# AlerianEmperor/CaitlynRenderer

Measured on AMD Instinct MI355X. Metric: Mray/s (primary+1 bounce) at 1920x1080, higher is better.
Workload: dtype f32

## Files before the change

### caitlynrenderer_amd/csrc/crt_device.cpp

```cpp
#include <hip/hip_runtime.h>
#include <dlfcn.h>

#include <algorithm>
#include <atomic>
#include <chrono>
#include <cmath>
#include <cstdio>
#include <cstdlib>
#include <cstring>
#include <memory>
#include <mutex>
#include <thread>
#include <new>
#include <string>
#include <vector>

#include "../../include/crt.h"
#include "crt_error.hpp"
#include "device_build.hpp"
#include "host/cwbvh.hpp"
#include "host/flatnode_link.hpp"
#include "host/refit_core.hpp"
#include "instances.hpp"
#include "instances_bind.hpp"
// ... 426 lines not shown
}

static int init_scene_common(crt_scene* s, const crt_scene_desc* d) {
    if (hipGetDevice(&s->device) != hipSuccess) return (fail(CRT_ERR_HIP, "hipGetDevice failed"));
    hipDeviceProp_t prop;
    if (hipGetDeviceProperties(&prop, s->device) == hipSuccess) s->n_cu = prop.multiProcessorCount;
    if (const char* e = std::getenv("CRT_TIMING")) s->timing = (uint32_t)std::max(0, std::atoi(e));
    if (hipStreamCreateWithFlags(&s->stream, hipStreamNonBlocking) != hipSuccess) return (fail(CRT_ERR_HIP, "hipStreamCreate failed"));
    s->width = d->width; s->height = d->height; s->max_depth = d->max_depth; s->n_lights = (uint32_t)d->n_lights;
    s->n_vertices = d->n_vertices; s->n_normals = d->n_normals; s->n_slots = d->n_triangles;
    if (d->n_vertices) {
        for (int k = 0; k < 3; ++k) s->bounds_lo[k] = s->bounds_hi[k] = d->vertices[k];
        for (size_t i = 1; i < d->n_vertices; ++i)
            for (int k = 0; k < 3; ++k) {
                s->bounds_lo[k] = std::min(s->bounds_lo[k], d->vertices[3 * i + k]);
                s->bounds_hi[k] = std::max(s->bounds_hi[k], d->vertices[3 * i + k]);
            }
    }
    for (size_t m = 0; m < d->n_materials; ++m)
        s->special_materials = s->special_materials || d->materials[m].albedo[3] == 1.0f || d->materials[m].albedo[3] == 17.0f;
    return CRT_OK;
}

static void note_buf(crt_scene* s, const void* member, size_t bytes) {
    s->scene_bufs.emplace_back((size_t)(reinterpret_cast<const char*>(member) - reinterpret_cast<const char*>(s)), bytes);
}

template <typename T>
static int pad_rows(crt_scene* s, T** buf, uint32_t rows_in, uint32_t rows_out, size_t n_items) {
    if (rows_in == rows_out || !*buf) return CRT_OK;
    T* padded = nullptr;
    int rc = dev_alloc(&padded, n_items * rows_out);
    if (rc) return rc;
    crt::launch_restride(*buf, rows_in, padded, rows_out, n_items, s->stream);
    if (hipStreamSynchronize(s->stream) != hipSuccess || hipGetLastError() != hipSuccess) { (void)hipFree(padded); return fail(CRT_ERR_HIP, "crt_scene_create: re-striding failed"); }
    (void)hipFree(*buf);
    *buf = padded;
    return CRT_OK;
}

static int ensure_planes(crt_scene* s) {
    if (s->d_planes || !s->d_nodes || !s->info.n_nodes8) return CRT_OK;
    int rc;
    if (s->primary && s->shares_scene) {
        crt_scene* const p = s->primary;
        if ((rc = ensure_planes(p))) return rc;
// ... 311 lines not shown
    } else if (!nodes8) {
        if (!conv.convert(d->bvh, d->n_bvh, d->n_triangles, d->tri_orig_ids))
            return fail(CRT_ERR_INVALID, "crt_scene_create: BVH2 -> CWBVH failed: " + conv.error);
        nodes8 = conv.nodes.data(); n_nodes8 = conv.nodes.size();
        tri_slots = conv.tri_slots.data(); n_tris8 = conv.tri_slots.size();
    } else if (!tri_slots) {
        return fail(CRT_ERR_INVALID, "crt_scene_create: bvh8 given without bvh8_tri_slots");
    }
    {
        std::string why = crt::validate_cwbvh(nodes8, n_nodes8, n_tris8, CRT_STACK_ENTRIES, &depth8);
        if (!why.empty()) return fail(why.find("deeper") != std::string::npos ? CRT_ERR_LIMIT : CRT_ERR_INVALID,
                                      "crt_scene_create: CWBVH rejected: " + why);
        for (size_t i = 0; i < n_tris8; ++i)
            if (tri_slots[i] < 0 || (size_t)tri_slots[i] >= d->n_triangles)
                return fail(CRT_ERR_INVALID, "crt_scene_create: bvh8_tri_slots entry out of range");
    }

    if (n_nodes8 * (uint64_t)(CRT_NODE_ROWS * 16) >= (1ull << 32) || n_tris8 * (uint64_t)(CRT_TRI_ROWS * 16) >= (1ull << 32))
        return fail(CRT_ERR_LIMIT, "crt_scene_create: CWBVH node or triangle-record array of 4 GiB or more (53 M nodes / 89 M records)");
    std::unique_ptr<crt_scene> owner(new (std::nothrow) crt_scene);
    crt_scene* s = owner.get();
    if (!s) return fail(CRT_ERR_NOMEM, "crt_scene_create: out of memory");
    auto bail = [&](int code) { return code; };
    if ((rc = init_scene_common(s, d))) return bail(rc);
    s->stack_entries = std::min<uint32_t>(CRT_STACK_ENTRIES, std::max<uint32_t>(2, depth8 - 1u));
    s->info.n_nodes8 = n_nodes8; s->info.n_tris8 = n_tris8; s->info.n_bvh2_nodes = d->n_bvh; s->info.max_depth8 = depth8;

    std::vector<float4> recs(3 * n_tris8);
    for (size_t i = 0; i < n_tris8; ++i) {
        const int32_t slot = tri_slots[i];
        const crt_triangle& t = d->triangles[slot];
        const float* v0 = d->vertices + 3 * (size_t)t.v[0];
        const float* v1 = d->vertices + 3 * (size_t)t.v[1];
        const float* v2 = d->vertices + 3 * (size_t)t.v[2];
        const int32_t id = d->tri_orig_ids ? d->tri_orig_ids[slot] : slot;
        float4 a, b, c;
        a.x = v0[0]; a.y = v0[1]; a.z = v0[2]; std::memcpy(&a.w, &id, 4);
        b.x = v1[0] - v0[0]; b.y = v1[1] - v0[1]; b.z = v1[2] - v0[2]; std::memcpy(&b.w, &slot, 4);
        c.x = v2[0] - v0[0]; c.y = v2[1] - v0[1]; c.z = v2[2] - v0[2]; std::memcpy(&c.w, &t.v[3], 4);
        recs[3 * i] = a; recs[3 * i + 1] = b; recs[3 * i + 2] = c;
    }

#define UP(dst, src, count, T)                                                                             \
    do {                                                                                                   \
        if ((rc = dev_alloc(&(dst), (count)))) return bail(rc);                                            \
        if ((count) && hipMemcpy((dst), (src), (count) * sizeof(T), hipMemcpyHostToDevice) != hipSuccess)  \
            return bail(fail(CRT_ERR_HIP, "hipMemcpy H2D failed"));                                        \
// ... 60 lines not shown
    note_buf(s, &s->d_normals, d->n_normals * 3 * sizeof(float));
    note_buf(s, &s->d_materials, d->n_materials * sizeof(crt_material));
    note_buf(s, &s->d_lights, d->n_lights * sizeof(crt_light));
    if (have_tex) {
        note_buf(s, &s->d_texcoords, d->n_texcoords * sizeof(float2));
        note_buf(s, &s->d_textures, (size_t)d->tex_width * d->tex_height * d->n_textures * 3 * sizeof(float));
    }
    if (d->bvh) {
        note_buf(s, &s->d_bvh2, d->n_bvh * sizeof(crt_flatnode));
        note_buf(s, &s->d_tris2, d->n_triangles * 3 * sizeof(float4));
    }
    if ((rc = finish_scene_setup(s))) return bail(rc);
    *out = owner.release();
    return CRT_OK;
}

static int scene_create_device_built(const crt_scene_desc* d, crt_scene** out) {
    const auto t_begin = std::chrono::steady_clock::now();
    if (2ull * d->n_triangles >= crt::kMaxLinkBits) return fail(CRT_ERR_LIMIT, "crt_scene_create: more than 2^29 triangles");
    const bool have_tex = d->albedo_textures && d->n_textures > 0;
    std::unique_ptr<crt_scene> owner(new (std::nothrow) crt_scene);
    crt_scene* s = owner.get();
    if (!s) return fail(CRT_ERR_NOMEM, "crt_scene_create: out of memory");
    int rc = init_scene_common(s, d);
    if (rc) return rc;
    const uint32_t n = (uint32_t)d->n_triangles, n2 = 2u * n - 1u;
    hipStream_t st = s->stream;

    crt::DeviceArena arena;
    auto P = crt::DeviceArena::padded;
    const uint32_t gpu_build_flags = (d->build_flags & CRT_BUILD_SAH) ? (CRT_GPU_BUILD_SAH | (d->build_flags & 0xff00u))
                                     : (d->build_flags & CRT_BUILD_PLOC) ? (CRT_GPU_BUILD_PLOC | (d->build_flags & 0xff00u)) : 0u;
    const size_t tmp_bytes = std::max(crt::lbvh_tmp_bytes(n, gpu_build_flags), crt::cwbvh_tmp_bytes(n2, n));
    hipError_t he = arena.reserve(P((size_t)n * sizeof(crt_triangle)) + P(4) + P((size_t)n * 4) + P((size_t)n * 4) + tmp_bytes);
    if (he != hipSuccess) return fail(CRT_ERR_NOMEM, std::string("crt_scene_create: hipMalloc: ") + hipGetErrorString(he));
    crt_triangle* d_in = arena.take<crt_triangle>(n);
    uint32_t* d_flag = arena.take<uint32_t>(1);
    uint32_t* d_tri_order = arena.take<uint32_t>(n);
    int32_t* d_tri_slots = arena.take<int32_t>(n);
    const size_t persistent_mark = arena.used;

#define UPA(dst, src, count, T)                                                                                      \
    do {                                                                                                             \
        if ((rc = dev_alloc(&(dst), (count)))) return rc;                                                            \
        if ((count) && hipMemcpyAsync((dst), (src), (count) * sizeof(T), hipMemcpyHostToDevice, st) != hipSuccess)   \
            return fail(CRT_ERR_HIP, "hipMemcpy H2D failed");                                                        \
    } while (0)
// ... 1550 lines not shown
```

### caitlynrenderer_amd/csrc/rt_kernels.hip

```cpp
#include <hip/hip_runtime.h>
#include <hip/hip_ext.h>
#include <stdint.h>

#include <type_traits>
#include <stdlib.h>

#include <algorithm>

#include "rt_kernels.hpp"
#include "rt_math.hpp"
#include "host/flatnode_link.hpp"
#include "rt_traverse.hpp"

namespace crt {

#define CRT_INF 1e9f
#define CRT_EPS 1e-4f
#define CRT_PI 3.1415926f
#define CRT_PI2 6.2831853f


#ifdef CRT_ISA_MARKS
#define CRT_MARK(name) asm volatile("; CRT_MARK " name)
#else
#define CRT_MARK(name) ((void)0)
#endif

__device__ __forceinline__ void count_wave_step(uint32_t& c) {
    const unsigned long long m = __ballot(true);
    if ((int)(threadIdx.x & 63u) == __builtin_ctzll(m)) ++c;
}

__device__ unsigned long long* g_step_hist = nullptr;
__device__ uint32_t g_step_hist_mode = 0u;
__device__ __forceinline__ void hist_node_step(bool any, uint32_t nidx = 0u, uint32_t oct = 0u) {
    unsigned long long* const h = g_step_hist;
    if (h == nullptr) return;
    const unsigned long long m = __ballot(true);
    uint32_t n = (uint32_t)__builtin_popcountll(m);
    if (g_step_hist_mode) {
        const uint32_t key = (nidx << 3) | (oct & 7u);
        unsigned long long left = m;
        n = 0u;
        while (left) {
            const uint32_t k0 = (uint32_t)__shfl((int)key, __builtin_ctzll(left));
            left &= ~__ballot(key == k0);
            ++n;
        }
// ... 849 lines not shown
        const uint32_t v = static_chunk<true>(wid, nullptr, a.n, it);
        if (v == CRT_NO_WORK) break;
        const uint32_t i = dense_item(v, wave, lane);
        if (i >= a.n) continue;
        const float4 r0 = a.rays[2 * (size_t)i], r1 = a.rays[2 * (size_t)i + 1];
        HitState best;
        uint32_t nn = 0, nt = 0;
        const bool hit = traverse_bvh2<ANY, STATS>(a.nodes, a.tris, V3(r0.x, r0.y, r0.z), V3(r1.x, r1.y, r1.z), r0.w, a.tie, stk,
                                                   (int)a.stack_entries, a.overflow, best, nn, nt);
        float4 h;
        h.x = ANY ? 0.f : (hit ? best.t : 0.f);
        h.y = ANY ? 0.f : best.u;
        h.z = ANY ? 0.f : best.v;
        h.w = __int_as_float(ANY ? (hit ? 0 : -1) : best.id);
        a.hits[i] = h;
        if (STATS) a.stats[i] = ((nt > 65535u ? 65535u : nt) << 16) | (nn > 65535u ? 65535u : nn);
    }
}


__device__ __forceinline__ uint32_t wave_append(bool want, uint32_t* counter) {
    const unsigned long long m = __ballot(want);
    if (m == 0ull) return 0u;
    const uint32_t lane = threadIdx.x & 63u;
    const int leader = __builtin_ctzll(m);
    uint32_t base = 0;
    if ((int)lane == leader) base = atomicAdd(counter, (uint32_t)__builtin_popcountll(m));
    base = __shfl(base, leader);
    return base + (uint32_t)__builtin_popcountll(m & ((1ull << lane) - 1ull));
}

#include "rt_sort.hpp"

__device__ __forceinline__ uint32_t here(uint32_t uniform) { asm volatile("" : "+s"(uniform)); return uniform; }

__device__ __forceinline__ bool pixel_of(const FrameArgs& f, uint32_t i, uint32_t& px, uint32_t& py) {
    uint32_t t, bx, by;
    const uint32_t k = i & 63u;
    if (f.tile_log2) {
        const uint32_t s2 = 2u * f.tile_log2, sb = f.tile_log2 - 3u;
        t = i >> s2;
        const uint32_t blk = (i & ((1u << s2) - 1u)) >> 6;
        bx = blk & ((1u << sb) - 1u); by = blk >> sb;
    } else {
        const uint32_t tile_px = here(f.tile * f.tile);
        t = i / tile_px;
        const uint32_t blk = (i - t * tile_px) >> 6, blocks_per_row = here(f.tile >> 3);
        by = blk / blocks_per_row; bx = blk - by * blocks_per_row;
    }
    const uint2 txy = f.tile_xy[t];
    px = txy.x * f.tile + bx * 8u + (k & 7u);
    py = txy.y * f.tile + by * 8u + (k >> 3);
    return px < f.width && py < f.height;
}

__device__ __forceinline__ int wrap_i(int i, int n) { const int m = i % n; return m < 0 ? m + n : m; }
__device__ __forceinline__ vec3 sample_albedo(const SegmentArgs& a, float u, float v, int layer) {
    const int W = a.tex_width, H = a.tex_height;
    layer = layer < 0 ? 0 : layer > a.n_textures - 1 ? a.n_textures - 1 : layer;
    const float* img = a.textures + (size_t)layer * (size_t)W * (size_t)H * 3;
    const float x = u * (float)W - 0.5f, y = v * (float)H - 0.5f;
    float x0 = __builtin_floorf(x), y0 = __builtin_floorf(y);
    float fx = x - x0, fy = y - y0;
    if (!(__builtin_fabsf(x0) < 1e9f)) { x0 = 0.f; fx = 0.f; }
    if (!(__builtin_fabsf(y0) < 1e9f)) { y0 = 0.f; fy = 0.f; }
    const int i0 = wrap_i((int)x0, W), i1 = wrap_i((int)x0 + 1, W);
    const int j0 = wrap_i((int)y0, H), j1 = wrap_i((int)y0 + 1, H);
// ... 130 lines not shown
    b.ovf_base = k->bins_out.ovf_base; b.per_lane = k->bins_out.per_lane;
    for (int i = 0; i < 3; ++i) { b.origin[i] = k->bins_out.origin[i]; b.scale[i] = k->bins_out.scale[i]; }
    return b;
}
__device__ __forceinline__ KArgs kernarg_here() {
    KArgs p = (KArgs)__builtin_amdgcn_kernarg_segment_ptr();
    asm volatile("" : "+s"(p));
    return p;
}

#ifndef CRT_SEG_OCC
#define CRT_SEG_OCC 6
#endif
#ifndef CRT_SEG_OCC_DEFERRED
#define CRT_SEG_OCC_DEFERRED 8
#endif
#ifndef CRT_SEG_OCC_FIRST
#define CRT_SEG_OCC_FIRST 6
#endif
#ifndef CRT_SEG_OCC_BATCH
#define CRT_SEG_OCC_BATCH 5
#endif

template <bool FIRST, bool STATS, bool TEX, bool PRETRACED, bool INPLACE, bool BVH2 = false, bool MAT = false, bool BATCH = false, bool WIDE = false, bool ONE = false,
          bool INST = false>
__global__ void __launch_bounds__(CRT_TRACE_BLOCK, ((WIDE || ONE) ? CRT_SEG_OCC_FIRST : (BATCH || STATS) ? CRT_SEG_OCC_BATCH : (!FIRST && !INPLACE && !PRETRACED) ? CRT_SEG_OCC_DEFERRED : CRT_SEG_OCC)) k_segment(std::conditional_t<INST, InstSegmentArgs, SegmentArgs> a) {
    extern __shared__ uint2 s_lds[];
    constexpr bool UNI_K = FIRST;
    const bool wave_samples = BATCH && !WIDE && !ONE && a.wave_samples == 1u;
    const bool lane_samples = BATCH && (ONE || a.wave_samples == 2u);
    const WaveId wid = wave_id(wave_samples, lane_samples);
    const uint32_t lane = wid.lane, wave = wid.wave;
    const uint32_t wave_stride = (a.stack_entries + CRT_HIT_SLOTS) * 64u;
    uint2* stk = s_lds + (size_t)wid.lds_wave * wave_stride + lane;
    int* stk2 = reinterpret_cast<int*>(s_lds) + (size_t)wid.lds_wave * a.stack_entries2 * 64u + lane;
    const float4* const recs = BVH2 ? a.tris2 : a.tris;
    const FrameArgs& f = a.f;
    uint32_t nn = 0, nt = 0, nn_any = 0, nt_any = 0;
    uint32_t wn = 0, wt = 0, wn_any = 0, wt_any = 0;
    uint32_t n_hits = 0;
    uint32_t nu = 0, nu_any = 0;
    if (FIRST && a.zero_counts && blockIdx.x == 0)
        for (uint32_t i = threadIdx.x; i < a.n_zero; i += blockDim.x) a.zero_counts[i] = 0u;
    CRT_CHUNK_LOOP(it) {
        uint32_t v;
        if (!FIRST && a.bin_start) {
            const uint32_t n_chunks = queue_chunks(a.count_in[0]), per_group = (n_chunks + 7u) >> 3;
            const uint32_t grp = wid.vblock & 7u, c = (wid.vblock >> 3) + it * (wid.vgrid >> 3);
            v = (c < per_group && grp * per_group + c < n_chunks) ? (grp << 28) | (grp * per_group + c) : CRT_NO_WORK;
        } else {
            v = static_chunk<FIRST>(wid, a.count_in, f.n_local_pixels, it);
        }
        if (v == CRT_NO_WORK) break;
        const uint32_t g = v >> 28;
        uint32_t* const count_shadow = a.count_shadow + g * CRT_COUNTER_STRIDE;
        uint32_t* const count_next = a.count_next + g * CRT_COUNTER_STRIDE;
        float4* const shadow_q = a.shadow + 2 * (size_t)g * a.sub_capacity;
        float4* const next_q = a.rays_next + 2 * (size_t)g * a.sub_capacity;
        uint32_t e, n;
        uint32_t cost_tile = 0;
        bool cost_valid = false;
        uint32_t cost_t0 = 0;
        if (FIRST) {
            e = dense_item(v, wave, lane);
            if (lane_samples) {
                const uint32_t j = lane & 15u, q = wid.quadrant;
                e = dense_item(v, wave, 0u) + (((q >> 1) * 4u + (j >> 2)) * 8u + (q & 1u) * 4u + (j & 3u));
            }
            n = f.n_local_pixels;
            if (f.tile_order && e < n) {
                const uint32_t tile_px = f.tile * f.tile;
                const uint32_t slot = f.tile_log2 ? e >> (2u * f.tile_log2) : e / here(tile_px);
                cost_tile = f.tile_order[slot];
                e = cost_tile * tile_px + (e - slot * tile_px);
            }
            if (a.tile_cost) cost_t0 = __builtin_amdgcn_readfirstlane((uint32_t)__builtin_readcyclecounter());
            cost_tile = __builtin_amdgcn_readlane(cost_tile, 0);
            cost_valid = __builtin_amdgcn_readlane((uint32_t)(e < n), 0) != 0u;
        } else {
            e = ((v & 0x0fffffffu) * 4u + wave) * 64u + lane;
            n = a.bin_start ? a.count_in[0] : a.count_in[g * CRT_COUNTER_STRIDE];
        }
        const uint32_t ws_waves = blockDim.x >> 6;
        const uint32_t n_smp = (ONE || !BATCH) ? 1u : (wave_samples ? (a.n_samples + ws_waves - 1u) / ws_waves : lane_samples ? a.n_samples >> 2 : a.n_samples);
        const uint32_t e_of_chunk = e;
        for (uint32_t smp_it = 0; smp_it < n_smp; ++smp_it) {
        if (BATCH) { e = e_of_chunk; asm volatile("" : "+v"(e)); }
        const uint32_t smp = wave_samples ? smp_it * ws_waves + wid.lds_wave : lane_samples ? smp_it * 4u + (lane >> 4) : smp_it;
        float rv = BATCH ? a.rv_s[smp & 7u] : f.rv;
        if (lane_samples) {
            rv = a.rv_s[0];
            for (uint32_t k = 1; k < 8u; ++k) rv = smp == k ? a.rv_s[k] : rv;
        }
        bool active = e < n && (!wave_samples || smp < a.n_samples);
        uint32_t pix = 0;
        vec3 o = V3(0.f, 0.f, 0.f), d = V3(0.f, 0.f, 1.f);
        vec3 L = V3(0.f, 0.f, 0.f), T = V3(1.f, 1.f, 1.f);
        float prev_pdf = 1.0f, sx = 0.f, sy = 0.f;
        bool is_specular = true, true_area = false;
        uint32_t slot_mask = 0u;
        if (FIRST) {
            uint32_t px = 0, py = 0;
            pix = BATCH ? smp * f.n_local_pixels + e : e;
            active = active && pixel_of(f, e, px, py);
            sx = (float)px + 0.5f; sy = (float)py + 0.5f;
            const float W = (float)here(f.width), H = (float)here(f.height);
            float jx = 0.f, jy = 0.f;
            if (f.jitter) {
                const float r1 = 2.0f * shader_rand(sx, sy, rv);
                const float r2 = 2.0f * shader_rand(sx, sy, rv);
                jx = r1 < 1.0f ? sqrt_ieee(r1) - 1.0f : 1.0f - sqrt_ieee(2.0f - r1);
                jy = r2 < 1.0f ? sqrt_ieee(r2) - 1.0f : 1.0f - sqrt_ieee(2.0f - r2);
                jx = __fdiv_rn(jx, W * 0.5f);
                jy = __fdiv_rn(jy, H * 0.5f);
            }
            const float tx = __fdiv_rn((float)px + 0.5f, W), ty = __fdiv_rn((float)py + 0.5f, H);
            float dx = (2.0f * tx - 1.0f) + jx;
            float dy = (2.0f * ty - 1.0f) + jy;
            dx = dx * f.aspect_tan;
            dy = dy * f.tan_fov;
            const vec3 right = V3(f.cam_right[0], f.cam_right[1], f.cam_right[2]);
            const vec3 up = V3(f.cam_up[0], f.cam_up[1], f.cam_up[2]);
            const vec3 fwd = V3(f.cam_forward[0], f.cam_forward[1], f.cam_forward[2]);
            d = normalize((right * dx + up * dy) + fwd);
            o = V3(f.cam_pos[0], f.cam_pos[1], f.cam_pos[2]);
        } else if (active) {
            const float4* rq;
            if (a.bin_start) {
                CRT_MARK("loop_begin bins");
                rq = a.rays_in + 2 * (size_t)binned_entry(a.bin_start, a.bin_off_in, a.ovf_base_in, e);
                CRT_MARK("loop_end");
            } else {
                rq = a.rays_in + 2 * ((size_t)g * a.sub_capacity + e);
            }
            const float4 r0 = rq[0], r1 = rq[1];
            o = V3(r0.x, r0.y, r0.z); d = V3(r1.x, r1.y, r1.z);
            pix = __float_as_uint(r1.w);
        }

        HitState hit;
        hit.tri = -1;
        if (PRETRACED) {
            if (active) {
                const float4 h = a.hits_in[(size_t)g * a.sub_capacity + e];
                hit.t = h.x; hit.u = h.y; hit.v = h.z; hit.tri = __float_as_int(h.w);
            }
        } else if (BVH2) {
            if (active) traverse_bvh2<false, STATS>(a.nodes2, a.tris2, o, d, CRT_INF, a.tie, stk2, (int)a.stack_entries2, a.overflow, hit, nn, nt);
// ... 13 lines not shown
                for (uint32_t k = 1; k < 8u; ++k) rv = smp_of == k ? ka->rv_s[k] : rv;
            }
            const float4 Tp = ka->pb.T[pix];
            const float2 sd = ka->pb.seed[pix];
            if (INPLACE) { const float4 Lp = ka->pb.L[pix]; L = V3(Lp.x, Lp.y, Lp.z); prev_pdf = Lp.w; }
            else prev_pdf = ka->pb.L[pix].w;
            T = V3(Tp.x, Tp.y, Tp.z);
            is_specular = (__float_as_uint(Tp.w) & 1u) != 0u;
            true_area = (__float_as_uint(Tp.w) & 2u) != 0u;
            slot_mask = __float_as_uint(Tp.w) & 0xffffff00u;
            sx = sd.x; sy = sd.y;
        }
        auto contribute = [&](vec3 c) {
            if (INPLACE) L = L + c;
            else { ka->contrib[pix] = make_float4(c.x, c.y, c.z, 1.0f); slot_mask |= ka->slot_bit; }
        };
        bool emit_shadow = false, emit_next = false, finished = active, pending = false;
        float pend_pdf = 0.f;
        float4 sh0 = make_float4(0, 0, 0, 0), sh1 = sh0, sh2 = sh0, nx0 = sh0, nx1 = sh0;
        if (active && hit.tri >= 0) {
            CRT_MARK("shade_begin");
            if (STATS) ++n_hits;
            const float t = hit.t, bu = hit.u, bv = hit.v;
            const size_t rec_rows = BVH2 ? 3u : (size_t)CRT_TRI_ROWS;
            int slot, mtl;
            uint32_t inst_word = 0u, inst_id = 0u, normal0 = 0u, texcoord0 = 0u;
            if constexpr (INST) {
                inst_id = (uint32_t)a.hit_inst[(size_t)g * ka->sub_capacity + e];
                const uint2 iw = a.inst_mesh[inst_id];
                inst_word = iw.x;
                const uint4 mb = a.mesh_base[inst_word & 0x7fffffffu];
                slot = (int)mb.x + hit.tri;
                mtl = ka->triangles[3 * (size_t)slot].w + (int)iw.y;
                normal0 = mb.y; texcoord0 = mb.z;
            } else {
                const float4 tb = recs[rec_rows * (size_t)hit.tri + 1], tc = recs[rec_rows * (size_t)hit.tri + 2];
                slot = __float_as_int(tb.w); mtl = __float_as_int(tc.w);
            }
            int4 vn = ka->triangles[3 * (size_t)slot + 1];
            if constexpr (INST) { if (vn.w != 0) { vn.x += (int)normal0; vn.y += (int)normal0; vn.z += (int)normal0; } }
            vec3 n;
            if (vn.w == 0) n = V3((float)vn.x, (float)vn.y, (float)vn.z);
            else {
                const float* N = ka->normals;
                const vec3 na = V3(N[3 * (size_t)vn.x], N[3 * (size_t)vn.x + 1], N[3 * (size_t)vn.x + 2]);
                const vec3 nb = V3(N[3 * (size_t)vn.y], N[3 * (size_t)vn.y + 1], N[3 * (size_t)vn.y + 2]);
                const vec3 nc = V3(N[3 * (size_t)vn.z], N[3 * (size_t)vn.z + 1], N[3 * (size_t)vn.z + 2]);
                const float w = 1.0f - bu - bv;
                n = (na * w + nb * bu) + nc * bv;
            }
            if constexpr (INST) {
                if ((inst_word & 0x80000000u) == 0u) {
                    const float* W = a.inst_w2o + 12 * (size_t)inst_id;
                    vec3 m = V3((W[0] * n.x + W[4] * n.y) + W[8] * n.z, (W[1] * n.x + W[5] * n.y) + W[9] * n.z, (W[2] * n.x + W[6] * n.y) + W[10] * n.z);
                    const float ln = sqrt_ieee((n.x * n.x + n.y * n.y) + n.z * n.z), lm = sqrt_ieee((m.x * m.x + m.y * m.y) + m.z * m.z);
                    if (lm != 0.0f && __builtin_isfinite(lm)) m = m * __fdiv_rn(ln, lm);
                    n = m;
                }
            }
            const float4 m_albedo = ka->materials[4 * (size_t)mtl], m_emission = ka->materials[4 * (size_t)mtl + 1],
                         m_specular = ka->materials[4 * (size_t)mtl + 2];
            const float cos_incident = dot(d, n);
            const vec3 original_n = n;
            if (cos_incident > 0) n = -n;
            if (m_emission.w != -1.0f) {
                const vec3 em = V3(m_emission.x, m_emission.y, m_emission.z);
                if (is_specular) contribute(T * em);
                else {
                    vec3 ld = d * t;
                    const float len = length(ld);
                    ld = normalize(ld);
                    const float cos_light = -1.0f * dot(ld, n);
                    const float len2 = len * len;
                    const int li = (int)m_emission.w;
                    const float* ap = ka->lights + 18 * (size_t)li + 15;
                    float pdf_light = __fdiv_rn(len2, ap[0] * cos_light) * ap[1];
                    if (MAT && true_area) pdf_light = 2.0f * pdf_light;
                    const float tt = prev_pdf * prev_pdf;
                    const float w = __fdiv_rn(tt, pdf_light * pdf_light + tt);
                    contribute((T * em) * w);
                }
            } else {
                const vec3 hit_point = (o + d * t) + n * 0.0002f;
                vec3 albedo = V3(m_albedo.x, m_albedo.y, m_albedo.z);
                if (TEX) {
                    const float tex = ka->materials[4 * (size_t)mtl + 3].x;
                    if (tex != -1.0f && ka->textures != nullptr) {
                        int4 vt = ka->triangles[3 * (size_t)slot + 2];
                        if constexpr (INST) { vt.x += (int)texcoord0; vt.y += (int)texcoord0; vt.z += (int)texcoord0; }
                        const float2 ta = ka->texcoords[vt.x], tb2 = ka->texcoords[vt.y], tc2 = ka->texcoords[vt.z];
                        const float w = 1.0f - bu - bv;
                        const float tu = (ta.x * w + tb2.x * bu) + tc2.x * bv;
                        const float tv = (ta.y * w + tb2.y * bu) + tc2.y * bv;
                        const vec3 c = sample_albedo(a, tu, tv, (int)tex);
                        albedo = V3((float)pow((double)c.x, (double)2.2f), (float)pow((double)c.y, (double)2.2f),
                                    (float)pow((double)c.z, (double)2.2f));
                    }
                }
                const float mtype = m_albedo.w;
                if (MAT && mtype == CRT_MIRROR_TYPE) {
                    const vec3 ns = normalize(n);
                    const float dn = dot(d, ns);
                    T = T * albedo;
                    if (!ka->last_segment) {
                        const vec3 rdir = d - ns * (2.0f * dn);
                        if (INPLACE || FIRST) ka->pb.L[pix] = make_float4(L.x, L.y, L.z, prev_pdf);
                        ka->pb.T[pix] = make_float4(T.x, T.y, T.z, __uint_as_float(1u | slot_mask));
                        ka->pb.seed[pix] = make_float2(sx, sy);
                        emit_next = true;
                        finished = false;
                        nx0 = make_float4(hit_point.x, hit_point.y, hit_point.z, CRT_INF);
                        nx1 = make_float4(rdir.x, rdir.y, rdir.z, __uint_as_float(pix));
                    }
                } else {
                    const bool disney = MAT && mtype == CRT_DISNEY_TYPE;
                    vec3 ns = n;
                    const vec3 wo = -d;
                    Disney dm;
                    if (disney) { ns = normalize(n); dm = disney_params(albedo, m_specular.x, m_specular.y); }
                    if (m_specular.w == 0.0f) {
                        if (ka->n_lights <= 0) {
                            shader_rand(sx, sy, rv); shader_rand(sx, sy, rv); shader_rand(sx, sy, rv);
                        } else {
                            int li = (int)(shader_rand(sx, sy, rv) * (float)(int)here((uint32_t)ka->n_lights));
                            if (li > ka->n_lights - 1) li = ka->n_lights - 1;
                            const float* Lt = ka->lights + 18 * (size_t)li;
                            const float sq = sqrt_ieee(shader_rand(sx, sy, rv));
                            const float b0 = 1.0f - sq;
                            const float b1 = shader_rand(sx, sy, rv) * sq;
                            const vec3 lp = (V3(Lt[0], Lt[1], Lt[2]) + V3(Lt[3], Lt[4], Lt[5]) * b0) + V3(Lt[6], Lt[7], Lt[8]) * b1;
                            vec3 ldir = lp - hit_point;
                            const float len = length(ldir);
                            const float ilen = rcp_ieee(len);
                            ldir = ldir * ilen;
                            const float cos_mtl = dot(ldir, original_n);
                            const float cos_light = dot(ldir, V3(Lt[9], Lt[10], Lt[11]));
                            bool lit = cos_mtl > 0.0f && cos_light < 0.0f;
                            if (disney) lit = lit && dot(ns, ldir) > 0.0f;
                            if (lit) {
                                const vec3 le = V3(Lt[12], Lt[13], Lt[14]);
                                float pdf_light = __fdiv_rn(len * len, Lt[15] * -cos_light) * Lt[16];
                                vec3 c;
                                if (disney) {
                                    pdf_light = 2.0f * pdf_light;
                                    vec3 fr; float pdf_b;
                                    disney_eval(dm, ns, wo, ldir, fr, pdf_b);
                                    const float tt = pdf_light * pdf_light;
                                    const float w = __fdiv_rn(tt, pdf_b * pdf_b + tt);
                                    c = ((T * le) * fr) * (dot(ns, ldir) * w);
                                } else {
                                    const float bsdf_pdf = __fdiv_rn(dot(ldir, n) * 1.0f, CRT_PI);
                                    const float tt = pdf_light * pdf_light;
                                    const float w = __fdiv_rn(tt, bsdf_pdf * bsdf_pdf + tt);
                                    c = ((T * le) * albedo) * w;
                                }
                                c = V3(__fdiv_rn(c.x, pdf_light), __fdiv_rn(c.y, pdf_light), __fdiv_rn(c.z, pdf_light));
                                if (INPLACE) {
                                    const unsigned long long m = __ballot(true);
                                    if ((int)lane == __builtin_ctzll(m)) atomicAdd(count_shadow, (uint32_t)__builtin_popcountll(m));
                                    pending = true;
                                    sh2 = make_float4(c.x, c.y, c.z, 0.f);
                                } else {
                                    emit_shadow = true;
                                    contribute(c);
                                }
                                sh0 = make_float4(hit_point.x, hit_point.y, hit_point.z, len - CRT_EPS);
                                sh1 = make_float4(ldir.x, ldir.y, ldir.z, __uint_as_float(INPLACE ? pix : ka->slot_first + pix));
                            }
                        }
                    }
                    if (!ka->last_segment) {
                        vec3 sdir;
                        float bsdf_pdf;
                        bool go_on = true;
                        if (disney) {
                            const float u0 = shader_rand(sx, sy, rv);
                            const float u1 = shader_rand(sx, sy, rv);
                            const float u2 = shader_rand(sx, sy, rv);
                            sdir = disney_sample(dm, ns, wo, u0, u1, u2);
                            vec3 fr;
                            disney_eval(dm, ns, wo, sdir, fr, bsdf_pdf);
                            go_on = bsdf_pdf > 0.0f;
                            if (go_on) T = T * (fr * __fdiv_rn(dot(ns, sdir), bsdf_pdf));
                        } else {
                            vec3 ou, ov;
                            onb(n, ou, ov);
                            const float u1 = shader_rand(sx, sy, rv);
                            const float u2 = shader_rand(sx, sy, rv);
                            const float r = sqrt_ieee(u1);
                            const float phi = CRT_PI2 * u2;
                            const vec3 dl = V3(r * pinned_cos(phi), r * pinned_sin(phi), sqrt_ieee(1.0f - u1));
                            sdir = (ou * dl.x + ov * dl.y) + n * dl.z;
                            bsdf_pdf = __fdiv_rn(dot(sdir, n) * 1.0f, CRT_PI);
                            T = T * albedo;
                        }
                        if (go_on) {
                            if (INPLACE && pending) pend_pdf = bsdf_pdf;
                            else if (INPLACE || FIRST) ka->pb.L[pix] = make_float4(L.x, L.y, L.z, bsdf_pdf);
                            else reinterpret_cast<float*>(ka->pb.L + pix)[3] = bsdf_pdf;
                            ka->pb.T[pix] = make_float4(T.x, T.y, T.z, __uint_as_float((disney ? 2u : 0u) | slot_mask));
                            ka->pb.seed[pix] = make_float2(sx, sy);
                            emit_next = true;
                            finished = false;
                            nx0 = make_float4(hit_point.x, hit_point.y, hit_point.z, CRT_INF);
                            nx1 = make_float4(sdir.x, sdir.y, sdir.z, __uint_as_float(pix));
                        }
                    }
                }
            }
        }
        if (ka->bins_out.count) {
            const RayBins bins_out = load_bins(ka);
            CRT_MARK("loop_begin bins");
            uint32_t* const tab = wave_stride * 8u >= 3072u ? reinterpret_cast<uint32_t*>(s_lds + (size_t)wid.lds_wave * wave_stride) : nullptr;
            const uint32_t ni = bin_append(bins_out, emit_next, ray_bin_key(bins_out, nx0, nx1), tab);
            if (emit_next) { ka->rays_next[2 * (size_t)ni] = nx0; ka->rays_next[2 * (size_t)ni + 1] = nx1; }
            CRT_MARK("loop_end");
        } else {
            const uint32_t ni = wave_append(emit_next, count_next);
            if (emit_next) { next_q[2 * (size_t)ni] = nx0; next_q[2 * (size_t)ni + 1] = nx1; }
        }
        if (INPLACE) {
            const bool lanes_walks = !BVH2 && (ONE || (a.lanes_log2 != 0u && a.tri_min != 0u));
            if (FIRST && lanes_walks) {
                const bool occluded = traverse_any_then_groups<STATS, UNI_K>(a.nodes, a.tris, stk - lane, (int)a.stack_entries, a.overflow, pending, V3(sh0.x, sh0.y, sh0.z),
                                                                      V3(sh1.x, sh1.y, sh1.z), sh0.w, a.tri_min, a.lanes_log2, nn_any, nt_any, wn_any, wt_any, &nu_any, a.planes);
                if (pending && !occluded) L = L + V3(sh2.x, sh2.y, sh2.z);
            } else if (lanes_walks) {
                HitState shh;
                walk_batch<true, STATS, false, UNI_K>(a.nodes, a.tris, stk - lane, (int)a.stack_entries, a.overflow, pending, V3(sh0.x, sh0.y, sh0.z), V3(sh1.x, sh1.y, sh1.z),
                                               sh0.w, a.tri_min, a.lanes_log2, shh, nn_any, nt_any, wn_any, wt_any, V3(0.f, 0.f, 0.f), &nu_any, a.planes);
                if (pending && shh.tri < 0) L = L + V3(sh2.x, sh2.y, sh2.z);
            } else if (pending) {
                HitState sh;
                const vec3 so = V3(sh0.x, sh0.y, sh0.z), sd = V3(sh1.x, sh1.y, sh1.z);
                const bool occluded = BVH2
                    ? traverse_bvh2<true, STATS>(a.nodes2, a.tris2, so, sd, sh0.w, a.tie, stk2, (int)a.stack_entries2, a.overflow, sh, nn_any, nt_any)
                    : traverse<true, STATS, UNI_K>(a.nodes, a.tris, so, sd, sh0.w, stk, (int)a.stack_entries, a.overflow, sh, nn_any, nt_any, wn_any, wt_any, &nu_any);
                if (!occluded) L = L + V3(sh2.x, sh2.y, sh2.z);
            }
            if (pending && emit_next) a.pb.L[pix] = make_float4(L.x, L.y, L.z, pend_pdf);
            pending = false;
        } else {
// ... 379 lines not shown
```

### caitlynrenderer_amd/csrc/rt_math.hpp

```cpp
#pragma once
#include <hip/hip_runtime.h>
#include <stdint.h>

namespace crt {

struct vec3 { float x, y, z; };

__device__ __forceinline__ vec3 V3(float x, float y, float z) { return vec3{x, y, z}; }
__device__ __forceinline__ vec3 operator+(vec3 a, vec3 b) { return {a.x + b.x, a.y + b.y, a.z + b.z}; }
__device__ __forceinline__ vec3 operator-(vec3 a, vec3 b) { return {a.x - b.x, a.y - b.y, a.z - b.z}; }
__device__ __forceinline__ vec3 operator*(vec3 a, vec3 b) { return {a.x * b.x, a.y * b.y, a.z * b.z}; }
__device__ __forceinline__ vec3 operator*(vec3 a, float s) { return {a.x * s, a.y * s, a.z * s}; }
__device__ __forceinline__ vec3 operator-(vec3 a) { return {-a.x, -a.y, -a.z}; }
__device__ __forceinline__ float dot(vec3 a, vec3 b) { return (a.x * b.x + a.y * b.y) + a.z * b.z; }
__device__ __forceinline__ vec3 cross(vec3 a, vec3 b) {
    return {a.y * b.z - a.z * b.y, a.z * b.x - a.x * b.z, a.x * b.y - a.y * b.x};
}
#if defined(__gfx950__)
#define CRT_FAST_RCP 1
#else
#define CRT_FAST_RCP 0
#endif
__device__ __forceinline__ float sqrt_ieee(float x) {
#if CRT_FAST_RCP
// ... 44 lines not shown
    p = fma_add_const(p, z, -1.0 / 1307674368000.0);
    p = fma_add_const(p, z, 1.0 / 6227020800.0);
    p = fma_add_const(p, z, -1.0 / 39916800.0);
    p = fma_add_const(p, z, 1.0 / 362880.0);
    p = fma_add_const(p, z, -1.0 / 5040.0);
    p = fma_add_const(p, z, 1.0 / 120.0);
    p = fma_add_const(p, z, -1.0 / 6.0);
    return __builtin_fma(r * z, p, r);
}
__device__ __forceinline__ double cos_poly(double r) {
    double z = r * r;
    double p = z * (1.0 / 1124000727777607680000.0) + (-1.0 / 2432902008176640000.0);
    p = fma_add_const(p, z, 1.0 / 6402373705728000.0);
    p = fma_add_const(p, z, -1.0 / 20922789888000.0);
    p = fma_add_const(p, z, 1.0 / 87178291200.0);
    p = fma_add_const(p, z, -1.0 / 479001600.0);
    p = fma_add_const(p, z, 1.0 / 3628800.0);
    p = fma_add_const(p, z, -1.0 / 40320.0);
    p = fma_add_const(p, z, 1.0 / 720.0);
    p = fma_add_const(p, z, -1.0 / 24.0);
    p = fma_add_const(p, z, 0.5);
    return __builtin_fma(-z, p, 1.0);
}
__device__ __forceinline__ float pinned_sin(float xf) {
    double x = (double)xf;
    if (!(__builtin_fabs(x) < 1e9)) return 0.0f;
    double k, r = reduce_pi(x, k);
    double s = sin_poly(r);
    if (((long long)k) & 1) s = -s;
    return (float)s;
}
__device__ __forceinline__ float pinned_cos(float xf) {
    double x = (double)xf;
    if (!(__builtin_fabs(x) < 1e9)) return 1.0f;
    double k, r = reduce_pi(x, k);
    double c = cos_poly(r);
    if (((long long)k) & 1) c = -c;
    return (float)c;
}

__device__ __forceinline__ float shader_rand(float& sx, float& sy, float rv) {
    sx -= rv;
    sy -= rv;
    float d = sx * 12.9898f + sy * 78.233f;
    float v = pinned_sin(d) * 43758.5453f;
    return v - __builtin_floorf(v);
}

}
```

### caitlynrenderer_amd/csrc/rt_traverse.hpp

```cpp
#pragma once
#include <hip/hip_runtime.h>
#include <stdint.h>

#include "rt_kernels.hpp"
#include "rt_math.hpp"

namespace crt {

__device__ __forceinline__ uint32_t sign_extend_s8x4(uint32_t x) { return ((x >> 7) & 0x01010101u) * 0xffu; }


__device__ __forceinline__ float ubyte_f(uint32_t x, int j) { return (float)((x >> (8 * j)) & 0xffu); }

__device__ __forceinline__ uint32_t node8_intersect(const uint4 n0, const uint4 n1, const uint4 n2, const uint4 n3,
                                                    const uint4 n4, vec3 o, vec3 inv, bool negx, bool negy, bool negz,
                                                    uint32_t oct4, float max_t, uint32_t keep = 0xffu) {
    const vec3 p = V3(__uint_as_float(n0.x), __uint_as_float(n0.y), __uint_as_float(n0.z));
    const uint32_t e_imask = n0.w;
    const vec3 adj_inv = V3(__uint_as_float((e_imask & 0xffu) << 23) * inv.x,
                            __uint_as_float(((e_imask >> 8) & 0xffu) << 23) * inv.y,
                            __uint_as_float(((e_imask >> 16) & 0xffu) << 23) * inv.z);
    const vec3 adj_o = (p - o) * inv;
    uint32_t hit_mask = 0;
#pragma unroll
// ... 39 lines not shown
    const vec3 v0 = V3(a.x, a.y, a.z), e1 = V3(b.x, b.y, b.z), e2 = V3(c.x, c.y, c.z);
    const vec3 pv = cross(d, e2);
    const vec3 tv = o - v0;
    const vec3 qv = cross(tv, e1);
    float uu = dot(tv, pv);
    float vv = dot(d, qv);
    float tt = dot(e2, qv);
    const float inv_det = rcp_ieee(dot(e1, pv));
    uu = uu * inv_det;
    vv = vv * inv_det;
    tt = tt * inv_det;
    const float w = 1.0f - uu - vv;
    u = uu; v = vv; t = tt;
    return (uu >= 0.0f) & (vv >= 0.0f) & (tt >= 0.0f) & (w >= 0.0f);
}

__device__ __forceinline__ const uint4* node_rows(const uint4* nodes, uint32_t idx) {
    return reinterpret_cast<const uint4*>(reinterpret_cast<const char*>(nodes) + (size_t)(idx * (uint32_t)(CRT_NODE_ROWS * 16)));
}
__device__ __forceinline__ const float4* tri_rows(const float4* tris, uint32_t idx) {
    return reinterpret_cast<const float4*>(reinterpret_cast<const char*>(tris) + (size_t)(idx * (uint32_t)(CRT_TRI_ROWS * 16)));
}

#define CRT_COUNTER_STRIDE 32u


#ifdef CRT_EXPERIMENTS
#define CRT_CHUNK_LOOP(it) for (uint32_t it = 0;; ++it)
#else
#define CRT_CHUNK_LOOP(it) for (uint32_t it = 0; it < 1u; ++it)
#endif
#define CRT_NO_WORK 0xffffffffu

__device__ __forceinline__ uint32_t dense_chunks_of_group(uint32_t n_items, uint32_t g) {
    const uint32_t n_units = (((n_items + 63u) >> 6) + 63u) >> 6;
    return n_units > g ? ((n_units - g + 7u) >> 3) * 16u : 0u;
}
__device__ __forceinline__ uint32_t queue_chunks(uint32_t n) { return (((n + 63u) >> 6) + 3u) >> 2; }

struct WaveId { uint32_t lane, wave, lds_wave, vblock, vgrid, quadrant, sub; };
__device__ __forceinline__ WaveId wave_id(bool one_batch_per_workgroup = false, bool four_per_batch = false, uint32_t sub_log2 = 0u) {
    WaveId w;
    w.lane = threadIdx.x & 63u;
    w.lds_wave = threadIdx.x >> 6;
    w.sub = 0u;
    if (four_per_batch) {
// ... 52 lines not shown
```

Measured before the change: 17230.

## Tighten shading address math, skip append on last segment, add ISA marks

```diff
diff --git a/caitlynrenderer_amd/csrc/crt_device.cpp b/caitlynrenderer_amd/csrc/crt_device.cpp
--- a/caitlynrenderer_amd/csrc/crt_device.cpp
+++ b/caitlynrenderer_amd/csrc/crt_device.cpp
@@ -472,6 +472,14 @@
     return CRT_OK;
 }
 
+static int shading_arrays_addressable(const crt_scene_desc* d) {
+    const uint64_t limit = 1ull << 32;
+    if ((uint64_t)d->n_triangles * sizeof(crt_triangle) >= limit || (uint64_t)d->n_triangles * (CRT_TRI_ROWS * 16) >= limit ||
+        (uint64_t)d->n_normals * 12u >= limit || (uint64_t)d->n_materials * sizeof(crt_material) >= limit || (uint64_t)d->n_lights * sizeof(crt_light) >= limit)
+        return fail(CRT_ERR_LIMIT, "crt_scene_create: triangle, normal, material or light array of 4 GiB or more (89 M triangles, 357 M normals, 67 M materials, 59 M lights)");
+    return CRT_OK;
+}
+
 static void note_buf(crt_scene* s, const void* member, size_t bytes) {
     s->scene_bufs.emplace_back((size_t)(reinterpret_cast<const char*>(member) - reinterpret_cast<const char*>(s)), bytes);
 }
@@ -829,7 +837,7 @@
     crt_scene* s = owner.get();
     if (!s) return fail(CRT_ERR_NOMEM, "crt_scene_create: out of memory");
     auto bail = [&](int code) { return code; };
-    if ((rc = init_scene_common(s, d))) return bail(rc);
+    if ((rc = shading_arrays_addressable(d)) || (rc = init_scene_common(s, d))) return bail(rc);
     s->stack_entries = std::min<uint32_t>(CRT_STACK_ENTRIES, std::max<uint32_t>(2, depth8 - 1u));
     s->info.n_nodes8 = n_nodes8; s->info.n_tris8 = n_tris8; s->info.n_bvh2_nodes = d->n_bvh; s->info.max_depth8 = depth8;
 
@@ -936,7 +944,8 @@
     std::unique_ptr<crt_scene> owner(new (std::nothrow) crt_scene);
     crt_scene* s = owner.get();
     if (!s) return fail(CRT_ERR_NOMEM, "crt_scene_create: out of memory");
-    int rc = init_scene_common(s, d);
+    int rc = shading_arrays_addressable(d);
+    if (!rc) rc = init_scene_common(s, d);
     if (rc) return rc;
     const uint32_t n = (uint32_t)d->n_triangles, n2 = 2u * n - 1u;
     hipStream_t st = s->stream;
diff --git a/caitlynrenderer_amd/csrc/rt_kernels.hip b/caitlynrenderer_amd/csrc/rt_kernels.hip
--- a/caitlynrenderer_amd/csrc/rt_kernels.hip
+++ b/caitlynrenderer_amd/csrc/rt_kernels.hip
@@ -22,8 +22,12 @@
 
 #ifdef CRT_ISA_MARKS
 #define CRT_MARK(name) asm volatile("; CRT_MARK " name)
+#define CRT_MARK_PIN(name, x) asm volatile("; CRT_MARK " name : "+v"(x))
+#define CRT_MARK_EXPR(name, x) ({ asm volatile("; CRT_MARK " name); (x); })
 #else
 #define CRT_MARK(name) ((void)0)
+#define CRT_MARK_PIN(name, x) ((void)0)
+#define CRT_MARK_EXPR(name, x) (x)
 #endif
 
 __device__ __forceinline__ void count_wave_step(uint32_t& c) {
@@ -919,12 +923,15 @@
 __device__ __forceinline__ uint32_t wave_append(bool want, uint32_t* counter) {
     const unsigned long long m = __ballot(want);
     if (m == 0ull) return 0u;
+    CRT_MARK("cold_begin queue_append");
     const uint32_t lane = threadIdx.x & 63u;
     const int leader = __builtin_ctzll(m);
     uint32_t base = 0;
     if ((int)lane == leader) base = atomicAdd(counter, (uint32_t)__builtin_popcountll(m));
     base = __shfl(base, leader);
-    return base + (uint32_t)__builtin_popcountll(m & ((1ull << lane) - 1ull));
+    const uint32_t at = base + (uint32_t)__builtin_popcountll(m & ((1ull << lane) - 1ull));
+    CRT_MARK("cold_end");
+    return at;
 }
 
 #include "rt_sort.hpp"
@@ -940,6 +947,7 @@
         const uint32_t blk = (i & ((1u << s2) - 1u)) >> 6;
         bx = blk & ((1u << sb) - 1u); by = blk >> sb;
     } else {
+        CRT_MARK("cold npot_tiles");
         const uint32_t tile_px = here(f.tile * f.tile);
         t = i / tile_px;
         const uint32_t blk = (i - t * tile_px) >> 6, blocks_per_row = here(f.tile >> 3);
@@ -1116,6 +1124,13 @@
 #define CRT_SEG_OCC_BATCH 5
 #endif
 
+__device__ __forceinline__ float shell_rand(float& sx, float& sy, float rv) {
+    CRT_MARK_PIN("rng_begin", sx);
+    float r = shader_rand(sx, sy, rv);
+    CRT_MARK_PIN("rng_end", r);
+    return r;
+}
+
 template <bool FIRST, bool STATS, bool TEX, bool PRETRACED, bool INPLACE, bool BVH2 = false, bool MAT = false, bool BATCH = false, bool WIDE = false, bool ONE = false,
           bool INST = false>
 __global__ void __launch_bounds__(CRT_TRACE_BLOCK, ((WIDE || ONE) ? CRT_SEG_OCC_FIRST : (BATCH || STATS) ? CRT_SEG_OCC_BATCH : (!FIRST && !INPLACE && !PRETRACED) ? CRT_SEG_OCC_DEFERRED : CRT_SEG_OCC)) k_segment(std::conditional_t<INST, InstSegmentArgs, SegmentArgs> a) {
@@ -1134,8 +1149,11 @@
     uint32_t wn = 0, wt = 0, wn_any = 0, wt_any = 0;
     uint32_t n_hits = 0;
     uint32_t nu = 0, nu_any = 0;
-    if (FIRST && a.zero_counts && blockIdx.x == 0)
+    if (FIRST && a.zero_counts && blockIdx.x == 0) {
+        CRT_MARK("cold_begin zero_counts");
         for (uint32_t i = threadIdx.x; i < a.n_zero; i += blockDim.x) a.zero_counts[i] = 0u;
+        CRT_MARK("cold_end");
+    }
     CRT_CHUNK_LOOP(it) {
         uint32_t v;
         if (!FIRST && a.bin_start) {
@@ -1164,7 +1182,7 @@
             n = f.n_local_pixels;
             if (f.tile_order && e < n) {
                 const uint32_t tile_px = f.tile * f.tile;
-                const uint32_t slot = f.tile_log2 ? e >> (2u * f.tile_log2) : e / here(tile_px);
+                const uint32_t slot = f.tile_log2 ? e >> (2u * f.tile_log2) : CRT_MARK_EXPR("cold npot_tiles", e / here(tile_px));
                 cost_tile = f.tile_order[slot];
                 e = cost_tile * tile_px + (e - slot * tile_px);
             }
@@ -1182,7 +1200,10 @@
         if (BATCH) { e = e_of_chunk; asm volatile("" : "+v"(e)); }
         const uint32_t smp = wave_samples ? smp_it * ws_waves + wid.lds_wave : lane_samples ? smp_it * 4u + (lane >> 4) : smp_it;
         float rv = BATCH ? a.rv_s[smp & 7u] : f.rv;
-        if (lane_samples) {
+        if (ONE) {
+            const float rv_lo = (lane & 16u) ? a.rv_s[1] : a.rv_s[0], rv_hi = (lane & 16u) ? a.rv_s[3] : a.rv_s[2];
+            rv = (lane & 32u) ? rv_hi : rv_lo;
+        } else if (lane_samples) {
             rv = a.rv_s[0];
             for (uint32_t k = 1; k < 8u; ++k) rv = smp == k ? a.rv_s[k] : rv;
         }
@@ -1194,6 +1215,7 @@
         bool is_specular = true, true_area = false;
         uint32_t slot_mask = 0u;
         if (FIRST) {
+            CRT_MARK("raygen_begin");
             uint32_t px = 0, py = 0;
             pix = BATCH ? smp * f.n_local_pixels + e : e;
             active = active && pixel_of(f, e, px, py);
@@ -1201,10 +1223,12 @@
             const float W = (float)here(f.width), H = (float)here(f.height);
             float jx = 0.f, jy = 0.f;
             if (f.jitter) {
-                const float r1 = 2.0f * shader_rand(sx, sy, rv);
-                const float r2 = 2.0f * shader_rand(sx, sy, rv);
-                jx = r1 < 1.0f ? sqrt_ieee(r1) - 1.0f : 1.0f - sqrt_ieee(2.0f - r1);
-                jy = r2 < 1.0f ? sqrt_ieee(r2) - 1.0f : 1.0f - sqrt_ieee(2.0f - r2);
+                const float r1 = 2.0f * shell_rand(sx, sy, rv);
+                const float r2 = 2.0f * shell_rand(sx, sy, rv);
+                const bool lo1 = r1 < 1.0f, lo2 = r2 < 1.0f;
+                const float q1 = sqrt_ieee(lo1 ? r1 : 2.0f - r1), q2 = sqrt_ieee(lo2 ? r2 : 2.0f - r2);
+                jx = lo1 ? q1 - 1.0f : 1.0f - q1;
+                jy = lo2 ? q2 - 1.0f : 1.0f - q2;
                 jx = __fdiv_rn(jx, W * 0.5f);
                 jy = __fdiv_rn(jy, H * 0.5f);
             }
@@ -1218,6 +1242,7 @@
             const vec3 fwd = V3(f.cam_forward[0], f.cam_forward[1], f.cam_forward[2]);
             d = normalize((right * dx + up * dy) + fwd);
             o = V3(f.cam_pos[0], f.cam_pos[1], f.cam_pos[2]);
+            CRT_MARK_PIN("raygen_end", d.x);
         } else if (active) {
             const float4* rq;
             if (a.bin_start) {
@@ -1277,7 +1302,6 @@
             CRT_MARK("shade_begin");
             if (STATS) ++n_hits;
             const float t = hit.t, bu = hit.u, bv = hit.v;
-            const size_t rec_rows = BVH2 ? 3u : (size_t)CRT_TRI_ROWS;
             int slot, mtl;
             uint32_t inst_word = 0u, inst_id = 0u, normal0 = 0u, texcoord0 = 0u;
             if constexpr (INST) {
@@ -1288,9 +1312,12 @@
                 slot = (int)mb.x + hit.tri;
                 mtl = ka->triangles[3 * (size_t)slot].w + (int)iw.y;
                 normal0 = mb.y; texcoord0 = mb.z;
+            } else if constexpr (BVH2) {
+                const float4 tb = recs[3 * (size_t)hit.tri + 1], tc = recs[3 * (size_t)hit.tri + 2];
+                slot = __float_as_int(tb.w); mtl = __float_as_int(tc.w);
             } else {
-                const float4 tb = recs[rec_rows * (size_t)hit.tri + 1], tc = recs[rec_rows * (size_t)hit.tri + 2];
-                slot = __float_as_int(tb.w); mtl = __float_as_int(tc.w);
+                const float4* const rec = tri_rows(recs, (uint32_t)hit.tri);
+                slot = __float_as_int(rec[1].w); mtl = __float_as_int(rec[2].w);
             }
             int4 vn = ka->triangles[3 * (size_t)slot + 1];
             if constexpr (INST) { if (vn.w != 0) { vn.x += (int)normal0; vn.y += (int)normal0; vn.z += (int)normal0; } }
@@ -1298,9 +1325,10 @@
             if (vn.w == 0) n = V3((float)vn.x, (float)vn.y, (float)vn.z);
             else {
                 const float* N = ka->normals;
-                const vec3 na = V3(N[3 * (size_t)vn.x], N[3 * (size_t)vn.x + 1], N[3 * (size_t)vn.x + 2]);
-                const vec3 nb = V3(N[3 * (size_t)vn.y], N[3 * (size_t)vn.y + 1], N[3 * (size_t)vn.y + 2]);
-                const vec3 nc = V3(N[3 * (size_t)vn.z], N[3 * (size_t)vn.z + 1], N[3 * (size_t)vn.z + 2]);
+                const float* const pa = INST ? N + 3 * (size_t)vn.x : at_offset32(N, (uint32_t)vn.x * 12u);
+                const float* const pb = INST ? N + 3 * (size_t)vn.y : at_offset32(N, (uint32_t)vn.y * 12u);
+                const float* const pc = INST ? N + 3 * (size_t)vn.z : at_offset32(N, (uint32_t)vn.z * 12u);
+                const vec3 na = V3(pa[0], pa[1], pa[2]), nb = V3(pb[0], pb[1], pb[2]), nc = V3(pc[0], pc[1], pc[2]);
                 const float w = 1.0f - bu - bv;
                 n = (na * w + nb * bu) + nc * bv;
             }
@@ -1313,12 +1341,13 @@
                     n = m;
                 }
             }
-            const float4 m_albedo = ka->materials[4 * (size_t)mtl], m_emission = ka->materials[4 * (size_t)mtl + 1],
-                         m_specular = ka->materials[4 * (size_t)mtl + 2];
+            const float4* const mrow = INST ? ka->materials + 4 * (size_t)mtl : at_offset32(ka->materials, (uint32_t)mtl * 64u);
+            const float4 m_albedo = mrow[0], m_emission = mrow[1], m_specular = mrow[2];
             const float cos_incident = dot(d, n);
             const vec3 original_n = n;
             if (cos_incident > 0) n = -n;
             if (m_emission.w != -1.0f) {
+                CRT_MARK("cold_begin emissive_hit");
                 const vec3 em = V3(m_emission.x, m_emission.y, m_emission.z);
                 if (is_specular) contribute(T * em);
                 else {
@@ -1328,18 +1357,20 @@
                     const float cos_light = -1.0f * dot(ld, n);
                     const float len2 = len * len;
                     const int li = (int)m_emission.w;
-                    const float* ap = ka->lights + 18 * (size_t)li + 15;
+                    const float* ap = (INST ? ka->lights + 18 * (size_t)li : at_offset32(ka->lights, (uint32_t)li * 72u)) + 15;
                     float pdf_light = __fdiv_rn(len2, ap[0] * cos_light) * ap[1];
                     if (MAT && true_area) pdf_light = 2.0f * pdf_light;
                     const float tt = prev_pdf * prev_pdf;
                     const float w = __fdiv_rn(tt, pdf_light * pdf_light + tt);
                     contribute((T * em) * w);
                 }
+                CRT_MARK("cold_end");
             } else {
                 const vec3 hit_point = (o + d * t) + n * 0.0002f;
                 vec3 albedo = V3(m_albedo.x, m_albedo.y, m_albedo.z);
                 if (TEX) {
-                    const float tex = ka->materials[4 * (size_t)mtl + 3].x;
+                    CRT_MARK("cold_begin tex");
+                    const float tex = mrow[3].x;
                     if (tex != -1.0f && ka->textures != nullptr) {
                         int4 vt = ka->triangles[3 * (size_t)slot + 2];
                         if constexpr (INST) { vt.x += (int)texcoord0; vt.y += (int)texcoord0; vt.z += (int)texcoord0; }
@@ -1351,9 +1382,11 @@
                         albedo = V3((float)pow((double)c.x, (double)2.2f), (float)pow((double)c.y, (double)2.2f),
                                     (float)pow((double)c.z, (double)2.2f));
                     }
+                    CRT_MARK("cold_end");
                 }
                 const float mtype = m_albedo.w;
                 if (MAT && mtype == CRT_MIRROR_TYPE) {
+                    CRT_MARK("cold_begin mat");
                     const vec3 ns = normalize(n);
                     const float dn = dot(d, ns);
                     T = T * albedo;
@@ -1367,6 +1400,7 @@
                         nx0 = make_float4(hit_point.x, hit_point.y, hit_point.z, CRT_INF);
                         nx1 = make_float4(rdir.x, rdir.y, rdir.z, __uint_as_float(pix));
                     }
+                    CRT_MARK("cold_end");
                 } else {
                     const bool disney = MAT && mtype == CRT_DISNEY_TYPE;
                     vec3 ns = n;
@@ -1375,14 +1409,16 @@
                     if (disney) { ns = normalize(n); dm = disney_params(albedo, m_specular.x, m_specular.y); }
                     if (m_specular.w == 0.0f) {
                         if (ka->n_lights <= 0) {
-                            shader_rand(sx, sy, rv); shader_rand(sx, sy, rv); shader_rand(sx, sy, rv);
+                            CRT_MARK("cold_begin no_lights");
+                            shell_rand(sx, sy, rv); shell_rand(sx, sy, rv); shell_rand(sx, sy, rv);
+                            CRT_MARK("cold_end");
                         } else {
-                            int li = (int)(shader_rand(sx, sy, rv) * (float)(int)here((uint32_t)ka->n_lights));
+                            int li = (int)(shell_rand(sx, sy, rv) * (float)(int)here((uint32_t)ka->n_lights));
                             if (li > ka->n_lights - 1) li = ka->n_lights - 1;
-                            const float* Lt = ka->lights + 18 * (size_t)li;
-                            const float sq = sqrt_ieee(shader_rand(sx, sy, rv));
+                            const float* Lt = INST ? ka->lights + 18 * (size_t)li : at_offset32(ka->lights, (uint32_t)li * 72u);
+                            const float sq = sqrt_ieee(shell_rand(sx, sy, rv));
                             const float b0 = 1.0f - sq;
-                            const float b1 = shader_rand(sx, sy, rv) * sq;
+                            const float b1 = shell_rand(sx, sy, rv) * sq;
                             const vec3 lp = (V3(Lt[0], Lt[1], Lt[2]) + V3(Lt[3], Lt[4], Lt[5]) * b0) + V3(Lt[6], Lt[7], Lt[8]) * b1;
                             vec3 ldir = lp - hit_point;
                             const float len = length(ldir);
@@ -1425,13 +1461,14 @@
                         }
                     }
                     if (!ka->last_segment) {
+                        CRT_MARK("cold_begin not_last_segment");
                         vec3 sdir;
                         float bsdf_pdf;
                         bool go_on = true;
                         if (disney) {
-                            const float u0 = shader_rand(sx, sy, rv);
-                            const float u1 = shader_rand(sx, sy, rv);
-                            const float u2 = shader_rand(sx, sy, rv);
+                            const float u0 = shell_rand(sx, sy, rv);
+                            const float u1 = shell_rand(sx, sy, rv);
+                            const float u2 = shell_rand(sx, sy, rv);
                             sdir = disney_sample(dm, ns, wo, u0, u1, u2);
                             vec3 fr;
                             disney_eval(dm, ns, wo, sdir, fr, bsdf_pdf);
@@ -1440,8 +1477,8 @@
                         } else {
                             vec3 ou, ov;
                             onb(n, ou, ov);
-                            const float u1 = shader_rand(sx, sy, rv);
-                            const float u2 = shader_rand(sx, sy, rv);
+                            const float u1 = shell_rand(sx, sy, rv);
+                            const float u2 = shell_rand(sx, sy, rv);
                             const float r = sqrt_ieee(u1);
                             const float phi = CRT_PI2 * u2;
                             const vec3 dl = V3(r * pinned_cos(phi), r * pinned_sin(phi), sqrt_ieee(1.0f - u1));
@@ -1460,20 +1497,26 @@
                             nx0 = make_float4(hit_point.x, hit_point.y, hit_point.z, CRT_INF);
                             nx1 = make_float4(sdir.x, sdir.y, sdir.z, __uint_as_float(pix));
                         }
+                        CRT_MARK("cold_end");
                     }
                 }
             }
+            CRT_MARK("shade_end");
         }
         if (ka->bins_out.count) {
+            CRT_MARK("cold_begin ray_bins");
             const RayBins bins_out = load_bins(ka);
             CRT_MARK("loop_begin bins");
             uint32_t* const tab = wave_stride * 8u >= 3072u ? reinterpret_cast<uint32_t*>(s_lds + (size_t)wid.lds_wave * wave_stride) : nullptr;
             const uint32_t ni = bin_append(bins_out, emit_next, ray_bin_key(bins_out, nx0, nx1), tab);
             if (emit_next) { ka->rays_next[2 * (size_t)ni] = nx0; ka->rays_next[2 * (size_t)ni + 1] = nx1; }
             CRT_MARK("loop_end");
-        } else {
+            CRT_MARK("cold_end");
+        } else if (!ka->last_segment) {
+            CRT_MARK("cold_begin not_last_segment");
             const uint32_t ni = wave_append(emit_next, count_next);
             if (emit_next) { next_q[2 * (size_t)ni] = nx0; next_q[2 * (size_t)ni + 1] = nx1; }
+            CRT_MARK("cold_end");
         }
         if (INPLACE) {
             const bool lanes_walks = !BVH2 && (ONE || (a.lanes_log2 != 0u && a.tri_min != 0u));
diff --git a/caitlynrenderer_amd/csrc/rt_math.hpp b/caitlynrenderer_amd/csrc/rt_math.hpp
--- a/caitlynrenderer_amd/csrc/rt_math.hpp
+++ b/caitlynrenderer_amd/csrc/rt_math.hpp
@@ -90,21 +90,18 @@
     p = fma_add_const(p, z, 0.5);
     return __builtin_fma(-z, p, 1.0);
 }
+__device__ __forceinline__ float negate_if_odd(float v, double k) {
+    return __uint_as_float(__float_as_uint(v) ^ ((uint32_t)(int)k << 31));
+}
 __device__ __forceinline__ float pinned_sin(float xf) {
-    double x = (double)xf;
-    if (!(__builtin_fabs(x) < 1e9)) return 0.0f;
-    double k, r = reduce_pi(x, k);
-    double s = sin_poly(r);
-    if (((long long)k) & 1) s = -s;
-    return (float)s;
+    if (!(__builtin_fabsf(xf) < 1e9f)) return 0.0f;
+    double k, r = reduce_pi((double)xf, k);
+    return negate_if_odd((float)sin_poly(r), k);
 }
 __device__ __forceinline__ float pinned_cos(float xf) {
-    double x = (double)xf;
-    if (!(__builtin_fabs(x) < 1e9)) return 1.0f;
-    double k, r = reduce_pi(x, k);
-    double c = cos_poly(r);
-    if (((long long)k) & 1) c = -c;
-    return (float)c;
+    if (!(__builtin_fabsf(xf) < 1e9f)) return 1.0f;
+    double k, r = reduce_pi((double)xf, k);
+    return negate_if_odd((float)cos_poly(r), k);
 }
 
 __device__ __forceinline__ float shader_rand(float& sx, float& sy, float rv) {
diff --git a/caitlynrenderer_amd/csrc/rt_traverse.hpp b/caitlynrenderer_amd/csrc/rt_traverse.hpp
--- a/caitlynrenderer_amd/csrc/rt_traverse.hpp
+++ b/caitlynrenderer_amd/csrc/rt_traverse.hpp
@@ -85,6 +85,11 @@
     return reinterpret_cast<const float4*>(reinterpret_cast<const char*>(tris) + (size_t)(idx * (uint32_t)(CRT_TRI_ROWS * 16)));
 }
 
+template <typename T>
+__device__ __forceinline__ const T* at_offset32(const T* base, uint32_t byte_offset) {
+    return reinterpret_cast<const T*>(reinterpret_cast<const char*>(base) + (size_t)byte_offset);
+}
+
 #define CRT_COUNTER_STRIDE 32u
 
 
```

New measurement: 17390, median of 6. No clear change (+0.9%).
